# hank-kuo-cs/Volumetric-Primitives-Net

Measured on AMD Instinct MI355X. Metric: render+Chamfer fwd+bwd images/sec, higher is better.
Workload: dtype f32; 1 GPU; C3: B=64/GPU (global 64), K=32 sphere primitives, 256x256 silhouette+depth, n=256 pts/prim (N=8192) vs M=2048 GT points, Chamfer+L1 fwd+bwd; global_batch=64, parallelism=dp1, collective=none, sampling=fresh Philox draws every step (device step counter, 28 steps drawn)

## Files before the change

volumetric-primitives-net_amd/csrc/chamfer.hip:

```cpp
#include "vpn_common.h"
#include "vpn_chamfer_feat.h"
#include "vpn_chamfer_loss.h"
#include "vpn_raster_common.h"
#include <stdlib.h>
#include <string.h>

#pragma clang fp contract(off)

namespace vpn {

constexpr int CH_BLOCK = 256;
constexpr int CH_WTILE = 256;

typedef float f2 __attribute__((ext_vector_type(2)));

#ifdef CM_EXP_TRACE
__device__ unsigned long long g_ctrace[8192 * 8];
extern "C" int vpn_debug_scan_trace(void* dst, int nwg) {
    return (int)hipMemcpyFromSymbol(dst, HIP_SYMBOL(g_ctrace), (size_t)nwg * 8 * sizeof(unsigned long long), 0, hipMemcpyDeviceToDevice);
}
#endif
#ifdef VPN_CHAMFER_DEBUG
__device__ unsigned long long g_dbg[8];
#endif

__device__ inline float dist2_exact(float ax, float ay, float az, float bx, float by, float bz) {
    float dx = ax - bx, dy = ay - by, dz = az - bz;
    return ((dx * dx) + (dy * dy)) + (dz * dz);
}

template <int R>
__global__ __launch_bounds__(CH_BLOCK) void chamfer_nn_kernel(const float* __restrict__ qpts,
                                                              const float* __restrict__ tpts, int Nq, int Nt,
                                                              float* __restrict__ out_dist,
                                                              int32_t* __restrict__ out_idx) {
    __shared__ __attribute__((aligned(16))) float lds[4][3][CH_WTILE];
    const int b = blockIdx.y;
    const int wave = threadIdx.x >> 6, lane = threadIdx.x & 63;
// ... 684 lines not shown
            for (int o = 32; o > 0; o >>= 1) l = min(l, __shfl_xor(l, o, 64));
            if (lane == 0) redi[c][wave] = l;
        }
        __syncthreads();
        if (threadIdx.x < CF_Q && k0 + (int)threadIdx.x < count) {
            const int c = threadIdx.x;
            float sc = s[0]; int qc = q[0];
#pragma unroll
            for (int e = 1; e < CF_Q; ++e) { sc = c == e ? s[e] : sc; qc = c == e ? q[e] : qc; }
            qc = min(max(qc, 0), Nq - 1);
            const int found = min(min(redi[c][0], redi[c][1]), min(redi[c][2], redi[c][3]));
            if (found != 0x7fffffff) {
                out_dist[(size_t)b * Nq + qc] = sc;
                out_idx[(size_t)b * Nq + qc] = found;
            }
        }
        __syncthreads();
    }
}

__device__ inline float vmin3(float a, float b, float c) {
    float r;
    asm("v_min3_f32 %0, %1, %2, %3" : "=v"(r) : "v"(a), "v"(b), "v"(c));
    return r;
}
__device__ inline float min16(const f16v& v) {
    const float a = __builtin_fminf(__builtin_fminf(v[0], v[1]), v[2]);
    const float b = __builtin_fminf(__builtin_fminf(v[3], v[4]), v[5]);
    const float c = __builtin_fminf(__builtin_fminf(v[6], v[7]), v[8]);
    const float d = __builtin_fminf(__builtin_fminf(v[9], v[10]), v[11]);
    const float e = __builtin_fminf(__builtin_fminf(v[12], v[13]), v[14]);
    const float g = vmin3(d, e, v[15]);
    return vmin3(vmin3(a, b, c), g, g);
}

__device__ inline float min32(const f16v& u, const f16v& v) {
    const float a = __builtin_fminf(__builtin_fminf(u[0], u[1]), u[2]);
    const float b = __builtin_fminf(__builtin_fminf(u[3], u[4]), u[5]);
    const float c = __builtin_fminf(__builtin_fminf(u[6], u[7]), u[8]);
    const float d = __builtin_fminf(__builtin_fminf(u[9], u[10]), u[11]);
    const float e = __builtin_fminf(__builtin_fminf(u[12], u[13]), u[14]);
    const float a2 = __builtin_fminf(__builtin_fminf(v[0], v[1]), v[2]);
    const float b2 = __builtin_fminf(__builtin_fminf(v[3], v[4]), v[5]);
    const float c2 = __builtin_fminf(__builtin_fminf(v[6], v[7]), v[8]);
    const float d2 = __builtin_fminf(__builtin_fminf(v[9], v[10]), v[11]);
    const float e2 = __builtin_fminf(__builtin_fminf(v[12], v[13]), v[14]);
    const float g = vmin3(d, e, u[15]), g2 = vmin3(d2, e2, v[15]);
    const float h = vmin3(a, b, c), h2 = vmin3(a2, b2, c2);
    return vmin3(vmin3(h, g, h2), g2, g2);
}

__device__ inline float near_error(float eps, float abs_eps, float na, float sna, float sm2, float E_cloud) {
    const float rb = (sna + sm2) * (1.0f + 2.0e-6f);
    const float nbn = rb * rb;
    const float En = (eps * (2.0f * sna * rb + nbn + na) + abs_eps * 1.7320509f * (sna + rb)) * (1.0f + 2.0e-6f);
    return fminf(En, E_cloud);
}
__device__ inline float sqrt_up(float x) { return __builtin_amdgcn_sqrtf(x) * (1.0f + 4.0e-7f) + 1.0e-18f; }


#ifndef CM_FQ
#define CM_FQ 4
#endif
#ifndef CM_FUN
#define CM_FUN 2
#endif
// ... 53 lines not shown
                            if (t[e] <= thr[c] && j < Nt) {
                                const float d = dist2_exact(-0.5f * mx[c], -0.5f * my[c], -0.5f * mz[c], xs[e], ys[e], zs[e]);
                                atomicMin(&key[c], ((unsigned long long)__float_as_uint(sqrtf(d)) << 32) | (unsigned)j);
                            }
                        }
                    }
                }
            }
        }
        __syncthreads();
        if (threadIdx.x < FQ) {
            const int k = k0 + threadIdx.x;
            const unsigned long long best = key[threadIdx.x];
            key[threadIdx.x] = ~0ull;
            if (k < count) {
                const int qc = min(max(lqi[k].x, 0), Nq - 1);
                const float df = best != ~0ull ? __uint_as_float((unsigned)(best >> 32)) : lqd[k].w;
                out_dist[qc] = df;
                out_idx[qc] = best != ~0ull ? (int)(unsigned)best : lqi[k].y;
                lqd[k].w = df;
            }
        }
    }
}

struct ScanJob {
    const float* qpts; const float* F; const unsigned short* H; const unsigned int* nmax;
    int Nq, Nt, Ntp, gx, G;
    float* out_dist; int32_t* out_idx;
    float* wgsum;
    const int32_t* qperm;
    const float* tboxes;
    int cand;
};

template <int PREC>
#ifndef CM_WAVES_PER_EU
#define CM_WAVES_PER_EU 6
#endif
__global__ __launch_bounds__(cm_block<PREC>(), PREC == 1 ? 5 : CM_WAVES_PER_EU) void chamfer_nn_mfma_kernel(
    const ScanJob j0, const ScanJob j1, int nsamples, const RasterOrderJob oj) {
    __shared__ __attribute__((aligned(16))) unsigned char tileH16[PREC == 2 ? 2 * CM_TILE16 * CM_ROWB : 16];
    if constexpr (PREC == 2) {
        if ((int)blockIdx.x < oj.B) {
            __builtin_amdgcn_s_setprio(3);
            raster_order_wg<cm_block<PREC>()>(oj, (int)blockIdx.x, tileH16);
            return;
        }
    }
    const int wg = (int)blockIdx.x - (PREC == 2 ? oj.B : 0);
#ifdef CM_EXP_TRACE
    const unsigned long long t_start = wall_clock64();
    unsigned long long t_pro = t_start;
#endif
    __shared__ int s_cnt;
    if (threadIdx.x == 0) s_cnt = 0;
    const bool other = wg >= j0.G;
    const float* __restrict__ qpts = other ? j1.qpts : j0.qpts;
    const float* __restrict__ F = other ? j1.F : j0.F;
    const unsigned short* __restrict__ H = other ? j1.H : j0.H;
    const unsigned int* __restrict__ nmax = other ? j1.nmax : j0.nmax;
    const int Nq = other ? j1.Nq : j0.Nq, Nt = other ? j1.Nt : j0.Nt, Ntp = other ? j1.Ntp : j0.Ntp;
    const int gx = other ? j1.gx : j0.gx, G = other ? j1.G : j0.G;
    float* __restrict__ out_dist = other ? j1.out_dist : j0.out_dist;
    int32_t* __restrict__ out_idx = other ? j1.out_idx : j0.out_idx;
    float* __restrict__ wgsum = other ? j1.wgsum : j0.wgsum;
    const int32_t* __restrict__ qperm = PREC == 2 ? (other ? j1.qperm : j0.qperm) : nullptr;
    const float* __restrict__ tboxes = PREC == 2 ? (other ? j1.tboxes : j0.tboxes) : nullptr;
    const int cand = PREC == 2 ? (other ? j1.cand : j0.cand) : 0;
    constexpr int QPW = cm_block<PREC>() / 2;
    constexpr int LISTB = QPW * 24 > (PREC == 2 ? 3 * CCAND_CAP * 4 : 0) ? QPW * 24 : 3 * CCAND_CAP * 4;
    __shared__ __attribute__((aligned(16))) unsigned char s_list[LISTB];
    float4* const s_qd = reinterpret_cast<float4*>(s_list);
    int2* const s_qi = reinterpret_cast<int2*>(s_list + QPW * 16);
    float* const s_cpl = reinterpret_cast<float*>(s_list);
    __shared__ unsigned short s_cidx[PREC == 2 ? CCAND_CAP : 2];
    int ccount = 0, cpad = 0;
    int vid = wg - (other ? j0.G : 0);
    {
        const int per = G >> 3;
        if (vid < (per << 3)) vid = (vid & 7) * per + (vid >> 3);
    }
    const int b = vid / gx, bx = vid - b * gx;
    const int wave = threadIdx.x >> 6, lane = threadIdx.x & 63, jq = lane & 31, half = lane >> 5;
    const float* qb = qpts + (size_t)b * Nq * 3;
    const int qi = (bx * (cm_block<PREC>() / 64) + wave) * 32 + jq;
    const int qc = qperm ? min(max(qperm[(size_t)b * ((Nq + 63) & ~63) + min(qi, Nq - 1)], 0), Nq - 1) : min(qi, Nq - 1);
    const F3 a3 = ld3(qb + qc * 3);
    const float ax = a3.x, ay = a3.y, az = a3.z;
    const float bq0 = half ? -2.0f * ay : -2.0f * ax;
    const float bq1 = half ? 1.0f : -2.0f * az;

    float best = __builtin_inff(), second = __builtin_inff();
    int blk = 0;
#define CM_SEL(dst, cond_mask, a, b) asm volatile("v_cndmask_b32 %0, %1, %2, %3" : "=v"(dst) : "v"(b), "v"(a), "s"(cond_mask))
#define CM_UPDATE(m, tb0)                                                                      \
    {                                                                                          \
        const int t_ = (tb0);                                                                  \
        unsigned long long k1_;                                                                \
        asm volatile("v_cmp_lt_f32 %0, %1, %2" : "=s"(k1_) : "v"(m), "v"(best));               \
        second = __builtin_amdgcn_fmed3f(best, second, (m));                                   \
        CM_SEL(blk, k1_, t_, blk);                                           \
// ... 54 lines not shown
#define CM_PAIR(oa, ob, J)                                                                     \
    {                                                                                          \
        CM_PRIO(1)                                                                             \
        const f16v accA = block(oa), accB = block(ob);                                         \
        CM_PRIO(0)                                                                             \
        const float mAB = min32(accA, accB);                                                   \
        CM_UPDATE_C(mAB, J)                                                                    \
    }
        float skipc = __builtin_inff();
        const float* __restrict__ tbox = tboxes ? tboxes + (size_t)b * (Ntp >> 5) * CFEAT_BOXF : nullptr;
        if (tbox) {
            const float nb0 = __uint_as_float(wave_max_bits(lane < CFEAT_SLOTS ? nmax[b * CFEAT_SLOTS + lane] : 0u));
            const float na0 = ax * ax + ay * ay + az * az;
            const float r = sqrt_up(na0) + sqrt_up(nb0), r2 = r * r;
            const float E0 = CM_EPS_F16 * r2 * (1.0f + 1.0e-6f) + 5.9604644775390625e-08f * 1.7320509f * r;
            if (nb0 <= CM_DOMAIN16 && na0 <= CM_DOMAIN16) skipc = (na0 + E0) + (3.0e-5f * r2 + 1.0e-30f);
        }
#define CM_SCAN_TILE(T, t0, nblk)                                                              \
    {                                                                                          \
        const float before = best;                                                             \
        float4 a0 = rd(T, 0), a1 = rd(T, 1), b0 = rd(T, 2), b1 = rd(T, 3);                     \
        CM_PAIR(a0, a1, 0)                                                                     \
        if (nblk > 2) {                                                                        \
            a0 = rd(T, 4); a1 = rd(T, 5);                                                      \
            CM_PAIR(b0, b1, 1)                                                                 \
            if (nblk > 4) {                                                                    \
                b0 = rd(T, 6); b1 = rd(T, 7);                                                  \
                CM_PAIR(a0, a1, 2)                                                             \
                if (nblk > 6) CM_PAIR(b0, b1, 3)                                               \
            }                                                                                  \
        }                                                                                      \
        blk = best < before ? (t0) + (blkc << 6) : blk;    \
    }
        int buf = 0, blkc = 0;
        if (cand) {
            __shared__ float s_cred[8][CM_WAVES16];
            __shared__ int s_cwn[2][CM_WAVES16];
            const float inf = __builtin_inff();
            auto uni = [](float v) { return __int_as_float(__builtin_amdgcn_readfirstlane(__float_as_int(v))); };
            {
                const float l0 = feat_wave_minmax<false>(ax), l1 = feat_wave_minmax<false>(ay), l2 = feat_wave_minmax<false>(az);
                const float h0 = feat_wave_minmax<true>(ax), h1 = feat_wave_minmax<true>(ay), h2 = feat_wave_minmax<true>(az);
                if (lane == 0) {
                    s_cred[0][wave] = l0; s_cred[1][wave] = l1; s_cred[2][wave] = l2;
                    s_cred[3][wave] = h0; s_cred[4][wave] = h1; s_cred[5][wave] = h2;
                }
            }
            __syncthreads();
            float cc[3];
#pragma unroll
            for (int a = 0; a < 3; ++a) {
                float l = s_cred[a][0], h = s_cred[3 + a][0];
#pragma unroll
                for (int w = 1; w < CM_WAVES16; ++w) { l = fminf(l, s_cred[a][w]); h = fmaxf(h, s_cred[3 + a][w]); }
                cc[a] = uni((l + h) * 0.5f);
            }
            const int n4 = Ntp >> 2;
            const float4* f4 = reinterpret_cast<const float4*>(Fb);
            {
                float r2 = dist2_exact(ax, ay, az, cc[0], cc[1], cc[2]);
                r2 = r2 == r2 ? r2 : inf;
                float dmin = inf;
                for (int g = threadIdx.x; g < n4; g += CM_BLOCK16) {
                    const float4 X = f4[g], Y = f4[n4 + g], Z = f4[2 * n4 + g];
                    const float xs[4] = {X.x, X.y, X.z, X.w}, ys[4] = {Y.x, Y.y, Y.z, Y.w}, zs[4] = {Z.x, Z.y, Z.z, Z.w};
#pragma unroll
                    for (int e = 0; e < 4; ++e) {
                        const float d = dist2_exact(xs[e], ys[e], zs[e], cc[0], cc[1], cc[2]);
                        dmin = 4 * g + e < Nt ? fminf(dmin, d) : dmin;
                    }
                }
                r2 = feat_wave_minmax<true>(r2); dmin = feat_wave_minmax<false>(dmin);
                if (lane == 0) { s_cred[6][wave] = r2; s_cred[7][wave] = dmin; }
            }
            __syncthreads();
            float thr;
            {
                float r2 = s_cred[6][0], dc2 = s_cred[7][0];
#pragma unroll
                for (int w = 1; w < CM_WAVES16; ++w) { r2 = fmaxf(r2, s_cred[6][w]); dc2 = fminf(dc2, s_cred[7][w]); }
                const float R = (2.0f * sqrt_up(r2) + sqrt_up(dc2)) * (1.0f + 1.0e-6f);
                thr = uni((R * R) * (1.0f + CCAND_EPS) + CCAND_FLOOR);
            }
            int total = CCAND_CAP + 1;
            if (thr < inf) {
                total = 0;
                int pass = 0;
                for (int g0 = 0; g0 < n4; g0 += CM_BLOCK16, pass ^= 1) {
// ... 24 lines not shown
                                s_cpl[pos] = xs[e]; s_cpl[CCAND_CAP + pos] = ys[e]; s_cpl[2 * CCAND_CAP + pos] = zs[e];
                                const uint4* hr = reinterpret_cast<const uint4*>(Hb + (size_t)j * CM_ROWB16);
                                const uint4 r0 = hr[0], r1 = hr[1];
                                *reinterpret_cast<uint4*>(&tileH16[pos * CM_ROWB]) = r0;
                                *reinterpret_cast<uint4*>(&tileH16[pos * CM_ROWB + 16]) = r1;
                            }
                            ++pos;
                        }
                    }
                    total = __builtin_amdgcn_readfirstlane(total + all);
                    if (total > CCAND_CAP) break;
                }
            }
            if (total >= 1 && total <= CCAND_CAP) {
                ccount = total; cpad = (total + 63) & ~63;
                const int p = total + (int)threadIdx.x;
                if (p < cpad) {
                    const Row16 pad = sentinel_row16();
                    s_cidx[p] = 0;
                    s_cpl[p] = 0.0f; s_cpl[CCAND_CAP + p] = 0.0f; s_cpl[2 * CCAND_CAP + p] = 0.0f;
                    *reinterpret_cast<uint4*>(&tileH16[p * CM_ROWB]) = pad.lo;
                    *reinterpret_cast<uint4*>(&tileH16[p * CM_ROWB + 16]) = pad.hi;
                }
            }
            __syncthreads();
        }
#ifdef CM_EXP_TRACE
        t_pro = wall_clock64();
#endif
        if (cpad) {
            for (int t0 = 0; t0 < cpad; t0 += CM_TILE16) {
                const int nblk = min(CM_TILE16, cpad - t0) >> 5;
                const unsigned char* T = &tileH16[(t0 + jq) * CM_ROWB + half * 16];
                CM_SCAN_TILE(T, t0, nblk)
            }
        } else {
        Pre pre = fetch(0);
        stash(0, pre);
        __syncthreads();
        for (int t0 = 0; t0 < Ntp; t0 += CM_TILE16, buf ^= 1) {
            const bool more = t0 + CM_TILE16 < Ntp;
            if (more) pre = fetch(t0 + CM_TILE16);
            bool scan = true;
            if (tbox) {
                const float4 bl = *reinterpret_cast<const float4*>(tbox + (t0 >> 8) * CFEAT_BOXF);
                const float2 bh = *reinterpret_cast<const float2*>(tbox + (t0 >> 8) * CFEAT_BOXF + 4);
                const float dx = fmaxf(fmaxf(bl.x - ax, ax - bl.w), 0.0f);
                const float dy = fmaxf(fmaxf(bl.y - ay, ay - bh.x), 0.0f);
                const float dz = fmaxf(fmaxf(bl.z - az, az - bh.y), 0.0f);
                const float L = ((dx * dx + dy * dy) + dz * dz) * (1.0f - 1.0e-6f);
                scan = __ballot(!(L > __builtin_fmaf(best, CM_INV_S16SQ, skipc))) != 0ull;
#ifdef VPN_CHAMFER_DEBUG
                if (!scan && lane == 0) atomicAdd(&g_dbg[3], 1ull);
#endif
            }
            if (scan) {
            const int nblk = min(CM_TILE16, Ntp - t0) >> 5;
            const unsigned char* T = &tileH[buf][jq * CM_ROWB + half * 16];
            CM_SCAN_TILE(T, t0, nblk)
            }
            if (more) stash(buf ^ 1, pre);
            __syncthreads();
        }
        }
#undef CM_SCAN_TILE
#undef CM_PAIR
    } else     if constexpr (PREC == 1) {
        __shared__ __attribute__((aligned(16))) unsigned char tileH[2][CM_TILE16 * CM_ROWB];
        const unsigned char* Hb = reinterpret_cast<const unsigned char*>(H) + (size_t)b * Ntp * CM_ROWB;
        bf8 bqA;
        bs4 bqB;
        {
            unsigned short qx[3], qy[3], qz[3];
            split3_bf16(-2.0f * ax, qx); split3_bf16(-2.0f * ay, qy); split3_bf16(-2.0f * az, qz);
            auto slot = [&](int k) -> unsigned short {
                const int c = k / 6, t = k % 6;
                const int pi = (t == 1 || t == 5) ? 1 : (t == 3 ? 2 : 0);
                if (k < 18) {
                    const unsigned short v0 = c == 0 ? qx[0] : (c == 1 ? qy[0] : qz[0]);
                    const unsigned short v1 = c == 0 ? qx[1] : (c == 1 ? qy[1] : qz[1]);
                    const unsigned short v2 = c == 0 ? qx[2] : (c == 1 ? qy[2] : qz[2]);
                    return pi == 0 ? v0 : (pi == 1 ? v1 : v2);
                }
                return k < 21 ? (unsigned short)0x3F80 : (unsigned short)0;
            };
            us8 ua;
            us4 ub;
#pragma unroll
            for (int e = 0; e < 8; ++e) ua[e] = half ? slot(8 + e) : slot(e);
#pragma unroll
            for (int e = 0; e < 4; ++e) ub[e] = half ? slot(20 + e) : slot(16 + e);
            bqA = __builtin_bit_cast(bf8, ua); bqB = __builtin_bit_cast(bs4, ub);
        }
        constexpr int F4 = CM_TILE16 * CM_ROWB / 16 / CM_BLOCK;
        static_assert(F4 == 3, "tile fetch is written for 3 float4 per lane");
        const float4* Hq = reinterpret_cast<const float4*>(Hb) + threadIdx.x;
        struct Pre { float4 a, b, c; };
// ... 70 lines not shown
        }
    };
    float4 pre[CM_F4];
    fetch(0, pre);
    stash(0, pre);
    __syncthreads();
    int buf = 0;
    for (int t0 = 0; t0 < Ntp; t0 += CM_TILE, buf ^= 1) {
        const bool more = t0 + CM_TILE < Ntp;
        if (more) fetch(t0 + CM_TILE, pre);
        const int nblk = min(CM_TILE, Ntp - t0) >> 5;
        const float* T0 = &tileF[buf][half][jq];
        const float* T1 = &tileF[buf][2 + half][jq];
        float o0 = T0[0], o1 = T1[0], o2 = T0[32], o3 = T1[32];
        for (int u = 0; u < nblk; u += 2) {
            const float c0 = o0, c1 = o1, c2 = o2, c3 = o3;
            if (u + 2 < nblk) { o0 = T0[u * 32 + 64]; o1 = T1[u * 32 + 64]; o2 = T0[u * 32 + 96]; o3 = T1[u * 32 + 96]; }
            f16v accA = __builtin_amdgcn_mfma_f32_32x32x2f32(c0, bq0, zero, 0, 0, 0);
            f16v accB = __builtin_amdgcn_mfma_f32_32x32x2f32(c2, bq0, zero, 0, 0, 0);
            accA = __builtin_amdgcn_mfma_f32_32x32x2f32(c1, bq1, accA, 0, 0, 0);
            accB = __builtin_amdgcn_mfma_f32_32x32x2f32(c3, bq1, accB, 0, 0, 0);
            const float mA = min16(accA);
            CM_UPDATE(mA, t0 + u * 32)
            const float mB = min16(accB);
            CM_UPDATE(mB, t0 + u * 32 + 32)
        }
        if (more) stash(buf ^ 1, pre);
        __syncthreads();
    }
    }
#ifdef CM_EXP_TRACE
    const unsigned long long t_loop = wall_clock64();
#endif
    constexpr int CM_CELL = PREC == 2 ? 64 : 32;
    constexpr int NT = CM_CELL / 4;
    int K, hw;
    float Bv, V2;
    {
        const float ob = __shfl_xor(best, 32, 64), os = __shfl_xor(second, 32, 64);
        const int ok = __shfl_xor(blk, 32, 64);
        const bool mine = best < ob || (best == ob && (blk < ok || (blk == ok && half == 0)));
        Bv = mine ? best : ob;
        K = mine ? blk : ok;
        hw = mine ? half : half ^ 1;
        V2 = mine ? fminf(second, ob) : fminf(os, best);
    }
    float d2[NT];
    float m2 = __builtin_inff();
#ifdef VPN_CHAMFER_DEBUG
    if (K < 0 || K + CM_CELL > Ntp || (K & (CM_CELL - 1))) atomicAdd(&g_dbg[7], 1ull);
#endif
    const int nreal = cpad ? ccount : Nt;
    K = min(max(K, 0), (cpad ? cpad : Ntp) - CM_CELL);
    const int base = K + half * (2 * NT) + 4 * hw;
    {
        float4 X[NT / 4], Y[NT / 4], Z[NT / 4];
#pragma unroll
        for (int v = 0; v < NT / 4; ++v) {
            if (PREC == 2 && cpad) {
                X[v] = *reinterpret_cast<const float4*>(s_cpl + base + 8 * v);
                Y[v] = *reinterpret_cast<const float4*>(s_cpl + CCAND_CAP + base + 8 * v);
                Z[v] = *reinterpret_cast<const float4*>(s_cpl + 2 * CCAND_CAP + base + 8 * v);
            } else {
                X[v] = *reinterpret_cast<const float4*>(Fb + base + 8 * v);
                Y[v] = *reinterpret_cast<const float4*>(Fb + (size_t)Ntp + base + 8 * v);
                Z[v] = *reinterpret_cast<const float4*>(Fb + 2 * (size_t)Ntp + base + 8 * v);
            }
        }
#pragma unroll
        for (int v = 0; v < NT / 4; ++v) {
            const float xs[4] = {X[v].x, X[v].y, X[v].z, X[v].w}, ys[4] = {Y[v].x, Y[v].y, Y[v].z, Y[v].w};
            const float zs[4] = {Z[v].x, Z[v].y, Z[v].z, Z[v].w};
#pragma unroll
            for (int w = 0; w < 4; ++w) d2[v * 4 + w] = dist2_exact(ax, ay, az, xs[w], ys[w], zs[w]);
        }
        if (__ballot(K + CM_CELL > nreal)) {
#pragma unroll
            for (int e = 0; e < NT; ++e) d2[e] += (base + 8 * (e >> 2) + (e & 3) < nreal) ? 0.0f : __builtin_inff();
        }
#pragma unroll
        for (int e = 0; e < NT; ++e) m2 = fminf(m2, d2[e]);
    }
    m2 = fminf(m2, __shfl_xor(m2, 32, 64));
    static_assert(CFEAT_SLOTS <= 64, "one slot per lane");
    const float nb = __uint_as_float(wave_max_bits(lane < CFEAT_SLOTS ? nmax[b * CFEAT_SLOTS + lane] : 0u));
    const float na = ax * ax + ay * ay + az * az;
    const float sna = sqrt_up(na), snb = sqrt_up(nb);
    float E = (PREC == 2 ? CM_EPS_F16 : (PREC == 1 ? CM_EPS_BF16 : CM_EPS)) * (2.0f * sna * snb + nb + na) * (1.0f + 1.0e-6f);
    if (PREC == 2) {
        E += 5.9604644775390625e-08f * 1.7320509f * (sna + snb);
        Bv *= CM_INV_S16SQ; V2 *= CM_INV_S16SQ;
    }
    const float s = sqrtf(m2);
    const float band = E + 4.0e-6f * (m2 + na);
    const float band_near = near_error(PREC == 2 ? CM_EPS_F16 : (PREC == 1 ? CM_EPS_BF16 : CM_EPS), PREC == 2 ? 5.9604644775390625e-08f : 0.0f,
                                       na, sna, s * (1.0f + 1.0e-7f), E) + (4.0e-6f * m2 + 4.0e-7f * na);
    bool ambiguous = !(V2 > (m2 - na) + band_near) || !(m2 - na <= Bv + band);
    if (PREC == 2) ambiguous |= !(nb <= CM_DOMAIN16 && na <= CM_DOMAIN16);
    const float lim = m2 * (1.0f + 1.0e-6f);
    int li = NT;
#pragma unroll
    for (int e = NT - 1; e >= 0; --e)
        if (d2[e] == m2) li = e;
    int idx = li < NT ? base + 8 * (li >> 2) + (li & 3) : 0x7fffffff;
    bool near_tie;
    {
        const unsigned mb1 = __float_as_uint(m2) + 1u;
        unsigned gm = 0xffffffffu;
#pragma unroll
        for (int e = 0; e < NT; e += 2)
            gm = min(gm, min(__float_as_uint(d2[e]) - mb1, __float_as_uint(d2[e + 1]) - mb1));
        near_tie = m2 < __builtin_inff() && gm < __float_as_uint(lim) - __float_as_uint(m2);
    }
    if (__ballot(near_tie)) {
#pragma unroll
        for (int e = NT - 1; e >= 0; --e)
            if (d2[e] <= lim && sqrtf(d2[e]) == s) idx = min(idx, base + 8 * (e >> 2) + (e & 3));
    }
    idx = min(idx, __shfl_xor(idx, 32, 64));
    if (PREC == 2 && cpad) {
        idx = idx < cpad ? (int)s_cidx[idx] : idx;
        __syncthreads();
    }
    __shared__ float s_ws[cm_block<PREC>() / 64];
    int pos = -1;
    if (half == 0 && qi < Nq) {
        if (!ambiguous) {
            out_dist[(size_t)b * Nq + qc] = s;
            out_idx[(size_t)b * Nq + qc] = idx;
        } else {
            pos = atomicAdd(&s_cnt, 1);
            s_qd[pos] = make_float4(ax, ay, az, s); s_qi[pos] = make_int2(qc, idx);
#ifdef VPN_CHAMFER_DEBUG
            atomicAdd(&g_dbg[6], 1ull);
#endif
        }
    }
    __syncthreads();
    const int cnt = s_cnt;
#ifdef CM_EXP_TRACE
    const unsigned long long t_epi = wall_clock64();
#endif
    float sfin = (half == 0 && qi < Nq) ? s : 0.0f;
    if (cnt != 0) {
#ifdef VPN_CHAMFER_DEBUG
        const unsigned long long t_fix = wall_clock64();
#endif
        fixup_own<cm_block<PREC>()>(Fb, snb, Nq, Nt, Ntp, out_dist + (size_t)b * Nq, out_idx + (size_t)b * Nq, s_qd, s_qi, cnt);
        __syncthreads();
        if (pos >= 0) sfin = s_qd[pos].w;
#ifdef VPN_CHAMFER_DEBUG
        if (threadIdx.x == 0) {
            atomicAdd(&g_dbg[other ? 2 : 1], wall_clock64() - t_fix);
            atomicAdd(&g_dbg[other ? 5 : 4], 1ull);
        }
// ... 345 lines not shown
    w.undecided = reinterpret_cast<int*>(w.nmax + (size_t)B * CFEAT_SLOTS);
    w.perm = reinterpret_cast<int32_t*>(w.undecided + pad4(B) + 4 * (size_t)B * Nq);
    w.boxes = reinterpret_cast<float*>(w.perm + (size_t)B * w.Ntp);
    w.wgsum = w.boxes + (size_t)B * (w.Ntp / 32) * CS_BOXF;
    return w;
}

static int mfma_both(const float* p1, const float* p2, int B, int N, int M, float* ws, float* d1, int32_t* i1, float* d2,
                     int32_t* i2, int prec, hipStream_t s, bool features_ready = false,
                     const RasterOrderJob* rider = nullptr) {
    const bool fp32_filter = prec == 0;
    const MfmaWs w2 = mfma_carve(ws, B, M, N);
    const MfmaWs w1 = mfma_carve(ws + mfma_ws_floats(B, M, N), B, N, M);
    auto split = [](int Ntp) { return feat_split(Ntp); };
    const bool skip = prec == 2 && N >= CSKIP_MIN_TARGETS;
    auto cand = [&](int Nq, int Nt, const float* boxes) {
        return chamfer_cand() && prec == 2 && !boxes && Nq >= CSKIP_MIN_TARGETS && Nt <= CCAND_MAX_TARGETS ? 1 : 0;
    };
    const FeatJob f2{p2, M, w2.Ntp, split(w2.Ntp), w2.F, w2.nmax, fp32_filter ? nullptr : w2.H, prec == 2, nullptr,
                     skip ? w2.perm : nullptr};
    const FeatJob f1{p1, N, w1.Ntp, split(w1.Ntp), w1.F, w1.nmax, fp32_filter ? nullptr : w1.H, prec == 2,
                     skip ? w1.boxes : nullptr, nullptr};
    hipError_t e = hipSuccess;
    if (!features_ready) {
        const int ord = skip ? (B + 7) & ~7 : 0;
        VPN_LAUNCH(chamfer_feat_kernel, dim3(ord + B * (f2.ysplit + f1.ysplit)), dim3(CFEAT_THREADS), 0, s, f2, f1, B, ord);
        e = hipGetLastError();
        if (e != hipSuccess) return (int)e;
    }
    {
        const int qpw = prec == 2 ? 32 * CM_WAVES16 : 128;
        const int gx1 = (N + qpw - 1) / qpw, gx2 = (M + qpw - 1) / qpw;
        const ScanJob s1{p1, w2.F, w2.H, w2.nmax, N, M, w2.Ntp, gx1, gx1 * B, d1, i1, w2.wgsum, nullptr, nullptr,
                         cand(N, M, nullptr)};
        const ScanJob s2{p2, w1.F, w1.H, w1.nmax, M, N, w1.Ntp, gx2, gx2 * B, d2, i2, w1.wgsum,
                         f2.perm, f1.tboxes, cand(M, N, f1.tboxes)};
        const bool long_first = (long long)N > (long long)M;
        const ScanJob& ja = long_first ? s2 : s1;
        const ScanJob& jb = long_first ? s1 : s2;
        const RasterOrderJob none{};
        if (prec == 0)
            VPN_LAUNCH(chamfer_nn_mfma_kernel<0>, dim3(ja.G + jb.G), dim3(CM_BLOCK), 0, s, ja, jb, B, none);
        else if (prec == 1)
            VPN_LAUNCH(chamfer_nn_mfma_kernel<1>, dim3(ja.G + jb.G), dim3(CM_BLOCK), 0, s, ja, jb, B, none);
        else
            VPN_LAUNCH(chamfer_nn_mfma_kernel<2>, dim3(ja.G + jb.G + (rider ? rider->B : 0)), dim3(CM_BLOCK16), 0, s, ja, jb, B,
                       rider ? *rider : none);
        e = hipGetLastError();
        if (e != hipSuccess) return (int)e;
    }
    return 0;
}

static int chamfer_mode();
int chamfer_feat_jobs(void* workspace, size_t workspace_bytes, int B, int N, int M, const float* p1, const float* p2,
                      FeatJob* job1, FeatJob* job2) {
    if (!workspace || B <= 0 || N <= 0 || M <= 0 || ((uintptr_t)workspace & 15) != 0) return VPN_E_BADARG;
    if (workspace_bytes < vpn_chamfer_workspace(B, N, M)) return VPN_E_BADARG;
    const int forced = chamfer_mode();
    if (!(forced == 6 || (forced == 0 && (long)N * M >= 512L * 512L))) return VPN_E_BADARG;
    float* ws = (float*)workspace;
    const MfmaWs w2 = mfma_carve(ws, B, M, N);
    const MfmaWs w1 = mfma_carve(ws + mfma_ws_floats(B, M, N), B, N, M);
    const bool skip = N >= CSKIP_MIN_TARGETS;
    *job2 = FeatJob{p2, M, w2.Ntp, feat_split(w2.Ntp), w2.F, w2.nmax, w2.H, 1, nullptr, skip ? w2.perm : nullptr};
    *job1 = FeatJob{p1, N, w1.Ntp, feat_split(w1.Ntp), w1.F, w1.nmax, w1.H, 1, skip ? w1.boxes : nullptr, nullptr};
    return 0;
}

// ... 222 lines not shown
```

volumetric-primitives-net_amd/csrc/vpn_chamfer_feat.h:

```cpp
#pragma once
#include "vpn_common.h"

namespace vpn {

constexpr int CM_ROWB = 48;
__device__ inline void split3_bf16(float x, unsigned short p[3]) {
#pragma clang fp contract(off)
    const unsigned u0 = __float_as_uint(x);
    p[0] = (unsigned short)(u0 >> 16);
    const float r1 = x - __uint_as_float(u0 & 0xFFFF0000u);
    const unsigned u1 = __float_as_uint(r1);
    p[1] = (unsigned short)(u1 >> 16);
    const float r2 = r1 - __uint_as_float(u1 & 0xFFFF0000u);
    p[2] = (unsigned short)(__float_as_uint(r2) >> 16);
}

constexpr float CM_S16 = 2048.0f;
constexpr int CM_ROWB16 = 32;
__device__ inline void split2_f16(float X, _Float16 h[2]) {
    h[0] = (_Float16)X;
    h[1] = (_Float16)(X - (float)h[0]);
}

struct Row16 { uint4 lo, hi; };
// ... 80 lines not shown
}

__device__ inline void feat_finish_slice(const FeatJob& J, int b, int by, float nv, float* red) {
    if (by == 0 && (int)threadIdx.x >= J.ysplit && threadIdx.x < CFEAT_SLOTS) J.nmax[b * CFEAT_SLOTS + threadIdx.x] = 0u;
    nv = feat_wave_max(nv);
    if ((threadIdx.x & 63) == 0) red[threadIdx.x >> 6] = nv;
    __syncthreads();
    if (threadIdx.x == 0) {
        float m = red[0];
        for (int w = 1; w < CFEAT_THREADS / 64; ++w) m = fmaxf(m, red[w]);
        J.nmax[b * CFEAT_SLOTS + by] = __float_as_uint(m);
    }
}

template <bool MAX>
__device__ inline float feat_wave_minmax(float v) {
#define VPN_FDPP(v, ctrl, rmask) \
    __int_as_float(__builtin_amdgcn_update_dpp(__float_as_int(v), __float_as_int(v), ctrl, rmask, 0xf, false))
#define VPN_FOP(a, b) (MAX ? fmaxf(a, b) : fminf(a, b))
    v = VPN_FOP(v, VPN_FDPP(v, 0x111, 0xf)); v = VPN_FOP(v, VPN_FDPP(v, 0x112, 0xf));
    v = VPN_FOP(v, VPN_FDPP(v, 0x114, 0xf)); v = VPN_FOP(v, VPN_FDPP(v, 0x118, 0xf));
    v = VPN_FOP(v, VPN_FDPP(v, 0x142, 0xa)); v = VPN_FOP(v, VPN_FDPP(v, 0x143, 0xc));
#undef VPN_FOP
#undef VPN_FDPP
    return __int_as_float(__builtin_amdgcn_readlane(__float_as_int(v), 63));
}

constexpr int CFEAT_TILE = 256;
constexpr int CFEAT_BOXF = 8;
constexpr int CSKIP_MIN_TARGETS = 4096;
constexpr int CORD_MAX = 2048;
constexpr int CCAND_CAP = 512;
constexpr int CCAND_MAX_TARGETS = 65535;

__device__ inline float* feat_tile_box(float* boxes, int Np, int b, int t) {
    return boxes + ((size_t)b * (Np >> 5) + t) * CFEAT_BOXF;
}

__device__ inline void feat_tile_boxes(const FeatJob& J, int b, int rlo, int rhi) {
    if (!J.tboxes || rlo >= rhi) return;
    const float* f = J.F + (size_t)b * 4 * J.Np;
    const int lane = threadIdx.x & 63, wave = threadIdx.x >> 6;
    const float inf = __builtin_inff();
    for (int t = rlo / CFEAT_TILE + wave; t * CFEAT_TILE < rhi; t += CFEAT_THREADS / 64) {
        const int r0 = t * CFEAT_TILE, r1 = min(r0 + CFEAT_TILE, J.Np);
        float lo[3] = {-inf, -inf, -inf}, hi[3] = {inf, inf, inf};
        if (r0 >= rlo && r1 <= rhi) {
            lo[0] = lo[1] = lo[2] = inf; hi[0] = hi[1] = hi[2] = -inf;
            const int rn = min(r1, J.N);
            for (int r = r0 + lane; r < rn; r += 64) {
                const float x = f[r], y = f[J.Np + r], z = f[2 * J.Np + r];
                lo[0] = fminf(lo[0], x); hi[0] = fmaxf(hi[0], x);
                lo[1] = fminf(lo[1], y); hi[1] = fmaxf(hi[1], y);
                lo[2] = fminf(lo[2], z); hi[2] = fmaxf(hi[2], z);
            }
#pragma unroll
            for (int a = 0; a < 3; ++a) { lo[a] = feat_wave_minmax<false>(lo[a]); hi[a] = feat_wave_minmax<true>(hi[a]); }
        }
        if (lane == 0) {
            float4* o = reinterpret_cast<float4*>(feat_tile_box(J.tboxes, J.Np, b, t));
            o[0] = make_float4(lo[0], lo[1], lo[2], hi[0]);
            o[1] = make_float4(hi[1], hi[2], 0.f, 0.f);
        }
    }
}

// ... 148 lines not shown
```

Measured before the change: 419,100 images/s.

## Refine candidate-path chamfer scan to 16-wide cells and reuse precomputed query boxes

In the candidate-list branch of the f16 MFMA chamfer kernel, the scan now records the best block at 16-target granularity (min8 quads) instead of 64, so the exact fp32 refinement step only rechecks a 16-point cell. The refinement code is wrapped in a templated lambda so the cell size can differ between the candidate and full-scan paths. The query bounding-box center now comes from precomputed tile boxes when available, which avoids six wave reductions and a block barrier. The cost is more per-block min reductions and more update branches during the scan, plus extra code size and register pressure.

```diff
diff --git a/volumetric-primitives-net_amd/csrc/chamfer.hip b/volumetric-primitives-net_amd/csrc/chamfer.hip
--- a/volumetric-primitives-net_amd/csrc/chamfer.hip
+++ b/volumetric-primitives-net_amd/csrc/chamfer.hip
@@ -4,6 +4,7 @@
 #include "vpn_raster_common.h"
 #include <stdlib.h>
 #include <string.h>
+#include <type_traits>
 
 #pragma clang fp contract(off)
 
@@ -754,6 +755,13 @@
     const float e = __builtin_fminf(__builtin_fminf(v[12], v[13]), v[14]);
     const float g = vmin3(d, e, v[15]);
     return vmin3(vmin3(a, b, c), g, g);
+}
+
+template <int O>
+__device__ inline float min8(const f16v& v) {
+    const float a = __builtin_fminf(__builtin_fminf(v[O], v[O + 1]), v[O + 2]);
+    const float b = __builtin_fminf(__builtin_fminf(v[O + 3], v[O + 4]), v[O + 5]);
+    return vmin3(a, b, __builtin_fminf(v[O + 6], v[O + 7]));
 }
 
 __device__ inline float min32(const f16v& u, const f16v& v) {
@@ -873,6 +881,7 @@
     const int32_t* qperm;
     const float* tboxes;
     int cand;
+    const float* qboxes;
 };
 
 template <int PREC>
@@ -909,6 +918,7 @@
     const int32_t* __restrict__ qperm = PREC == 2 ? (other ? j1.qperm : j0.qperm) : nullptr;
     const float* __restrict__ tboxes = PREC == 2 ? (other ? j1.tboxes : j0.tboxes) : nullptr;
     const int cand = PREC == 2 ? (other ? j1.cand : j0.cand) : 0;
+    const float* __restrict__ qboxes = PREC == 2 ? (other ? j1.qboxes : j0.qboxes) : nullptr;
     constexpr int QPW = cm_block<PREC>() / 2;
     constexpr int LISTB = QPW * 24 > (PREC == 2 ? 3 * CCAND_CAP * 4 : 0) ? QPW * 24 : 3 * CCAND_CAP * 4;
     __shared__ __attribute__((aligned(16))) unsigned char s_list[LISTB];
@@ -1029,28 +1039,68 @@
         }                                                                                      \
         blk = best < before ? (t0) + (blkc << 6) : blk;    \
     }
+#define CM_QUADS(oa, ob, J0, J1, J2, J3)                                                       \
+    {                                                                                          \
+        const f16v accA = block(oa), accB = block(ob);                                         \
+        const float q0 = min8<0>(accA), q1 = min8<8>(accA), q2 = min8<0>(accB), q3 = min8<8>(accB); \
+        CM_UPDATE_C(q0, J0)                                                                    \
+        CM_UPDATE_C(q1, J1)                                                                    \
+        CM_UPDATE_C(q2, J2)                                                                    \
+        CM_UPDATE_C(q3, J3)                                                                    \
+    }
+#define CM_SCAN_TILE_Q(T, t0, nblk)                                                            \
+    {                                                                                          \
+        const float before = best;                                                             \
+        float4 a0 = rd(T, 0), a1 = rd(T, 1), b0 = rd(T, 2), b1 = rd(T, 3);                     \
+        CM_QUADS(a0, a1, 0, 1, 2, 3)                                                           \
+        if (nblk > 2) {                                                                        \
+            a0 = rd(T, 4); a1 = rd(T, 5);                                                      \
+            CM_QUADS(b0, b1, 4, 5, 6, 7)                                                       \
+            if (nblk > 4) {                                                                    \
+                b0 = rd(T, 6); b1 = rd(T, 7);                                                  \
+                CM_QUADS(a0, a1, 8, 9, 10, 11)                                                 \
+                if (nblk > 6) CM_QUADS(b0, b1, 12, 13, 14, 15)                                 \
+            }                                                                                  \
+        }                                                                                      \
+        blk = best < before ? (t0) + (blkc << 4) : blk;    \
+    }
         int buf = 0, blkc = 0;
         if (cand) {
             __shared__ float s_cred[8][CM_WAVES16];
             __shared__ int s_cwn[2][CM_WAVES16];
             const float inf = __builtin_inff();
             auto uni = [](float v) { return __int_as_float(__builtin_amdgcn_readfirstlane(__float_as_int(v))); };
-            {
-                const float l0 = feat_wave_minmax<false>(ax), l1 = feat_wave_minmax<false>(ay), l2 = feat_wave_minmax<false>(az);
-                const float h0 = feat_wave_minmax<true>(ax), h1 = feat_wave_minmax<true>(ay), h2 = feat_wave_minmax<true>(az);
-                if (lane == 0) {
-                    s_cred[0][wave] = l0; s_cred[1][wave] = l1; s_cred[2][wave] = l2;
-                    s_cred[3][wave] = h0; s_cred[4][wave] = h1; s_cred[5][wave] = h2;
+            float cc[3];
+            bool boxed = false;
+            if (qboxes && !qperm) {
+                const float* qbox = qboxes + ((size_t)b * (((Nq + 63) & ~63) >> 5) + bx) * CFEAT_BOXF;
+                const float4 bl = *reinterpret_cast<const float4*>(qbox);
+                const float2 bh = *reinterpret_cast<const float2*>(qbox + 4);
+                const float lo[3] = {bl.x, bl.y, bl.z}, hi[3] = {bl.w, bh.x, bh.y};
+                boxed = true;
+#pragma unroll
+                for (int a = 0; a < 3; ++a) {
+                    boxed = boxed && fabsf(lo[a]) < inf && fabsf(hi[a]) < inf;
+                    cc[a] = uni((lo[a] + hi[a]) * 0.5f);
                 }
             }
-            __syncthreads();
-            float cc[3];
-#pragma unroll
-            for (int a = 0; a < 3; ++a) {
-                float l = s_cred[a][0], h = s_cred[3 + a][0];
-#pragma unroll
-                for (int w = 1; w < CM_WAVES16; ++w) { l = fminf(l, s_cred[a][w]); h = fmaxf(h, s_cred[3 + a][w]); }
-                cc[a] = uni((l + h) * 0.5f);
+            if (!boxed) {
+                {
+                    const float l0 = feat_wave_minmax<false>(ax), l1 = feat_wave_minmax<false>(ay), l2 = feat_wave_minmax<false>(az);
+                    const float h0 = feat_wave_minmax<true>(ax), h1 = feat_wave_minmax<true>(ay), h2 = feat_wave_minmax<true>(az);
+                    if (lane == 0) {
+                        s_cred[0][wave] = l0; s_cred[1][wave] = l1; s_cred[2][wave] = l2;
+                        s_cred[3][wave] = h0; s_cred[4][wave] = h1; s_cred[5][wave] = h2;
+                    }
+                }
+                __syncthreads();
+#pragma unroll
+                for (int a = 0; a < 3; ++a) {
+                    float l = s_cred[a][0], h = s_cred[3 + a][0];
+#pragma unroll
+                    for (int w = 1; w < CM_WAVES16; ++w) { l = fminf(l, s_cred[a][w]); h = fmaxf(h, s_cred[3 + a][w]); }
+                    cc[a] = uni((l + h) * 0.5f);
+                }
             }
             const int n4 = Ntp >> 2;
             const float4* f4 = reinterpret_cast<const float4*>(Fb);
@@ -1141,7 +1191,7 @@
             for (int t0 = 0; t0 < cpad; t0 += CM_TILE16) {
                 const int nblk = min(CM_TILE16, cpad - t0) >> 5;
                 const unsigned char* T = &tileH16[(t0 + jq) * CM_ROWB + half * 16];
-                CM_SCAN_TILE(T, t0, nblk)
+                CM_SCAN_TILE_Q(T, t0, nblk)
             }
         } else {
         Pre pre = fetch(0);
@@ -1172,6 +1222,8 @@
             __syncthreads();
         }
         }
+#undef CM_SCAN_TILE_Q
+#undef CM_QUADS
 #undef CM_SCAN_TILE
 #undef CM_PAIR
     } else     if constexpr (PREC == 1) {
@@ -1308,95 +1360,106 @@
 #ifdef CM_EXP_TRACE
     const unsigned long long t_loop = wall_clock64();
 #endif
-    constexpr int CM_CELL = PREC == 2 ? 64 : 32;
-    constexpr int NT = CM_CELL / 4;
-    int K, hw;
-    float Bv, V2;
-    {
-        const float ob = __shfl_xor(best, 32, 64), os = __shfl_xor(second, 32, 64);
-        const int ok = __shfl_xor(blk, 32, 64);
-        const bool mine = best < ob || (best == ob && (blk < ok || (blk == ok && half == 0)));
-        Bv = mine ? best : ob;
-        K = mine ? blk : ok;
-        hw = mine ? half : half ^ 1;
-        V2 = mine ? fminf(second, ob) : fminf(os, best);
-    }
-    float d2[NT];
-    float m2 = __builtin_inff();
-#ifdef VPN_CHAMFER_DEBUG
-    if (K < 0 || K + CM_CELL > Ntp || (K & (CM_CELL - 1))) atomicAdd(&g_dbg[7], 1ull);
-#endif
-    const int nreal = cpad ? ccount : Nt;
-    K = min(max(K, 0), (cpad ? cpad : Ntp) - CM_CELL);
-    const int base = K + half * (2 * NT) + 4 * hw;
-    {
-        float4 X[NT / 4], Y[NT / 4], Z[NT / 4];
-#pragma unroll
-        for (int v = 0; v < NT / 4; ++v) {
-            if (PREC == 2 && cpad) {
-                X[v] = *reinterpret_cast<const float4*>(s_cpl + base + 8 * v);
-                Y[v] = *reinterpret_cast<const float4*>(s_cpl + CCAND_CAP + base + 8 * v);
-                Z[v] = *reinterpret_cast<const float4*>(s_cpl + 2 * CCAND_CAP + base + 8 * v);
-            } else {
-                X[v] = *reinterpret_cast<const float4*>(Fb + base + 8 * v);
-                Y[v] = *reinterpret_cast<const float4*>(Fb + (size_t)Ntp + base + 8 * v);
-                Z[v] = *reinterpret_cast<const float4*>(Fb + 2 * (size_t)Ntp + base + 8 * v);
-            }
-        }
-#pragma unroll
-        for (int v = 0; v < NT / 4; ++v) {
-            const float xs[4] = {X[v].x, X[v].y, X[v].z, X[v].w}, ys[4] = {Y[v].x, Y[v].y, Y[v].z, Y[v].w};
-            const float zs[4] = {Z[v].x, Z[v].y, Z[v].z, Z[v].w};
-#pragma unroll
-            for (int w = 0; w < 4; ++w) d2[v * 4 + w] = dist2_exact(ax, ay, az, xs[w], ys[w], zs[w]);
-        }
-        if (__ballot(K + CM_CELL > nreal)) {
-#pragma unroll
-            for (int e = 0; e < NT; ++e) d2[e] += (base + 8 * (e >> 2) + (e & 3) < nreal) ? 0.0f : __builtin_inff();
-        }
-#pragma unroll
-        for (int e = 0; e < NT; ++e) m2 = fminf(m2, d2[e]);
-    }
-    m2 = fminf(m2, __shfl_xor(m2, 32, 64));
     static_assert(CFEAT_SLOTS <= 64, "one slot per lane");
     const float nb = __uint_as_float(wave_max_bits(lane < CFEAT_SLOTS ? nmax[b * CFEAT_SLOTS + lane] : 0u));
     const float na = ax * ax + ay * ay + az * az;
     const float sna = sqrt_up(na), snb = sqrt_up(nb);
-    float E = (PREC == 2 ? CM_EPS_F16 : (PREC == 1 ? CM_EPS_BF16 : CM_EPS)) * (2.0f * sna * snb + nb + na) * (1.0f + 1.0e-6f);
-    if (PREC == 2) {
-        E += 5.9604644775390625e-08f * 1.7320509f * (sna + snb);
-        Bv *= CM_INV_S16SQ; V2 *= CM_INV_S16SQ;
-    }
-    const float s = sqrtf(m2);
-    const float band = E + 4.0e-6f * (m2 + na);
-    const float band_near = near_error(PREC == 2 ? CM_EPS_F16 : (PREC == 1 ? CM_EPS_BF16 : CM_EPS), PREC == 2 ? 5.9604644775390625e-08f : 0.0f,
-                                       na, sna, s * (1.0f + 1.0e-7f), E) + (4.0e-6f * m2 + 4.0e-7f * na);
-    bool ambiguous = !(V2 > (m2 - na) + band_near) || !(m2 - na <= Bv + band);
-    if (PREC == 2) ambiguous |= !(nb <= CM_DOMAIN16 && na <= CM_DOMAIN16);
-    const float lim = m2 * (1.0f + 1.0e-6f);
-    int li = NT;
-#pragma unroll
-    for (int e = NT - 1; e >= 0; --e)
-        if (d2[e] == m2) li = e;
-    int idx = li < NT ? base + 8 * (li >> 2) + (li & 3) : 0x7fffffff;
-    bool near_tie;
-    {
-        const unsigned mb1 = __float_as_uint(m2) + 1u;
-        unsigned gm = 0xffffffffu;
-#pragma unroll
-        for (int e = 0; e < NT; e += 2)
-            gm = min(gm, min(__float_as_uint(d2[e]) - mb1, __float_as_uint(d2[e + 1]) - mb1));
-        near_tie = m2 < __builtin_inff() && gm < __float_as_uint(lim) - __float_as_uint(m2);
-    }
-    if (__ballot(near_tie)) {
+    float s;
+    int idx;
+    bool ambiguous;
+    auto finish = [&](auto cell) {
+        constexpr int CM_CELL = decltype(cell)::value;
+        constexpr int NT = CM_CELL / 4;
+        int K, hw;
+        float Bv, V2;
+        {
+            const float ob = __shfl_xor(best, 32, 64), os = __shfl_xor(second, 32, 64);
+            const int ok = __shfl_xor(blk, 32, 64);
+            const bool mine = best < ob || (best == ob && (blk < ok || (blk == ok && half == 0)));
+            Bv = mine ? best : ob;
+            K = mine ? blk : ok;
+            hw = mine ? half : half ^ 1;
+            V2 = mine ? fminf(second, ob) : fminf(os, best);
+        }
+        float d2[NT];
+        float m2 = __builtin_inff();
+#ifdef VPN_CHAMFER_DEBUG
+        if (K < 0 || K + CM_CELL > Ntp || (K & (CM_CELL - 1))) atomicAdd(&g_dbg[7], 1ull);
+#endif
+        const int nreal = cpad ? ccount : Nt;
+        K = min(max(K, 0), (cpad ? cpad : Ntp) - CM_CELL);
+        const int base = K + half * (2 * NT) + 4 * hw;
+        {
+            float4 X[NT / 4], Y[NT / 4], Z[NT / 4];
+#pragma unroll
+            for (int v = 0; v < NT / 4; ++v) {
+                if (PREC == 2 && cpad) {
+                    X[v] = *reinterpret_cast<const float4*>(s_cpl + base + 8 * v);
+                    Y[v] = *reinterpret_cast<const float4*>(s_cpl + CCAND_CAP + base + 8 * v);
+                    Z[v] = *reinterpret_cast<const float4*>(s_cpl + 2 * CCAND_CAP + base + 8 * v);
+                } else {
+                    X[v] = *reinterpret_cast<const float4*>(Fb + base + 8 * v);
+                    Y[v] = *reinterpret_cast<const float4*>(Fb + (size_t)Ntp + base + 8 * v);
+                    Z[v] = *reinterpret_cast<const float4*>(Fb + 2 * (size_t)Ntp + base + 8 * v);
+                }
+            }
+#pragma unroll
+            for (int v = 0; v < NT / 4; ++v) {
+                const float xs[4] = {X[v].x, X[v].y, X[v].z, X[v].w}, ys[4] = {Y[v].x, Y[v].y, Y[v].z, Y[v].w};
+                const float zs[4] = {Z[v].x, Z[v].y, Z[v].z, Z[v].w};
+#pragma unroll
+                for (int w = 0; w < 4; ++w) d2[v * 4 + w] = dist2_exact(ax, ay, az, xs[w], ys[w], zs[w]);
+            }
+            if (__ballot(K + CM_CELL > nreal)) {
+#pragma unroll
+                for (int e = 0; e < NT; ++e) d2[e] += (base + 8 * (e >> 2) + (e & 3) < nreal) ? 0.0f : __builtin_inff();
+            }
+#pragma unroll
+            for (int e = 0; e < NT; ++e) m2 = fminf(m2, d2[e]);
+        }
+        m2 = fminf(m2, __shfl_xor(m2, 32, 64));
+        float E = (PREC == 2 ? CM_EPS_F16 : (PREC == 1 ? CM_EPS_BF16 : CM_EPS)) * (2.0f * sna * snb + nb + na) * (1.0f + 1.0e-6f);
+        if (PREC == 2) {
+            E += 5.9604644775390625e-08f * 1.7320509f * (sna + snb);
+            Bv *= CM_INV_S16SQ; V2 *= CM_INV_S16SQ;
+        }
+        s = sqrtf(m2);
+        const float band = E + 4.0e-6f * (m2 + na);
+        const float band_near = near_error(PREC == 2 ? CM_EPS_F16 : (PREC == 1 ? CM_EPS_BF16 : CM_EPS), PREC == 2 ? 5.9604644775390625e-08f : 0.0f,
+                                           na, sna, s * (1.0f + 1.0e-7f), E) + (4.0e-6f * m2 + 4.0e-7f * na);
+        ambiguous = !(V2 > (m2 - na) + band_near) || !(m2 - na <= Bv + band);
+        if (PREC == 2) ambiguous |= !(nb <= CM_DOMAIN16 && na <= CM_DOMAIN16);
+        const float lim = m2 * (1.0f + 1.0e-6f);
+        int li = NT;
 #pragma unroll
         for (int e = NT - 1; e >= 0; --e)
-            if (d2[e] <= lim && sqrtf(d2[e]) == s) idx = min(idx, base + 8 * (e >> 2) + (e & 3));
-    }
-    idx = min(idx, __shfl_xor(idx, 32, 64));
-    if (PREC == 2 && cpad) {
-        idx = idx < cpad ? (int)s_cidx[idx] : idx;
-        __syncthreads();
+            if (d2[e] == m2) li = e;
+        idx = li < NT ? base + 8 * (li >> 2) + (li & 3) : 0x7fffffff;
+        bool near_tie;
+        {
+            const unsigned mb1 = __float_as_uint(m2) + 1u;
+            unsigned gm = 0xffffffffu;
+#pragma unroll
+            for (int e = 0; e < NT; e += 2)
+                gm = min(gm, min(__float_as_uint(d2[e]) - mb1, __float_as_uint(d2[e + 1]) - mb1));
+            near_tie = m2 < __builtin_inff() && gm < __float_as_uint(lim) - __float_as_uint(m2);
+        }
+        if (__ballot(near_tie)) {
+#pragma unroll
+            for (int e = NT - 1; e >= 0; --e)
+                if (d2[e] <= lim && sqrtf(d2[e]) == s) idx = min(idx, base + 8 * (e >> 2) + (e & 3));
+        }
+        idx = min(idx, __shfl_xor(idx, 32, 64));
+        if (PREC == 2 && cpad) {
+            idx = idx < cpad ? (int)s_cidx[idx] : idx;
+            __syncthreads();
+        }
+    };
+    if constexpr (PREC == 2) {
+        if (cpad) finish(std::integral_constant<int, CCAND_CELL>{});
+        else finish(std::integral_constant<int, 64>{});
+    } else {
+        finish(std::integral_constant<int, 32>{});
     }
     __shared__ float s_ws[cm_block<PREC>() / 64];
     int pos = -1;
@@ -1808,9 +1871,9 @@
         const int qpw = prec == 2 ? 32 * CM_WAVES16 : 128;
         const int gx1 = (N + qpw - 1) / qpw, gx2 = (M + qpw - 1) / qpw;
         const ScanJob s1{p1, w2.F, w2.H, w2.nmax, N, M, w2.Ntp, gx1, gx1 * B, d1, i1, w2.wgsum, nullptr, nullptr,
-                         cand(N, M, nullptr)};
+                         cand(N, M, nullptr), f1.tboxes};
         const ScanJob s2{p2, w1.F, w1.H, w1.nmax, M, N, w1.Ntp, gx2, gx2 * B, d2, i2, w1.wgsum,
-                         f2.perm, f1.tboxes, cand(M, N, f1.tboxes)};
+                         f2.perm, f1.tboxes, cand(M, N, f1.tboxes), nullptr};
         const bool long_first = (long long)N > (long long)M;
         const ScanJob& ja = long_first ? s2 : s1;
         const ScanJob& jb = long_first ? s1 : s2;
diff --git a/volumetric-primitives-net_amd/csrc/vpn_chamfer_feat.h b/volumetric-primitives-net_amd/csrc/vpn_chamfer_feat.h
--- a/volumetric-primitives-net_amd/csrc/vpn_chamfer_feat.h
+++ b/volumetric-primitives-net_amd/csrc/vpn_chamfer_feat.h
@@ -136,6 +136,7 @@
 constexpr int CORD_MAX = 2048;
 constexpr int CCAND_CAP = 512;
 constexpr int CCAND_MAX_TARGETS = 65535;
+constexpr int CCAND_CELL = 16;
 
 __device__ inline float* feat_tile_box(float* boxes, int Np, int b, int t) {
     return boxes + ((size_t)b * (Np >> 5) + t) * CFEAT_BOXF;
```

After: 439,100 images/s (median of 6 runs). 4.8% higher.
